# MarkJhonBao/InfantPoseEstimation_GaussianBias

Hardware: AMD Instinct MI355X
Metric: images/sec (train fwd+bwd) HRFormer-S 256x192 (higher is better)
Workload: dtype bf16; 1 GPU; HRFormer-small + fusion head, 256x192 -> 64x48, K=17, train step fwd+bwd+AdamW, DropPath 0.1, BN train; global_batch=64, per_gpu_batch=64, parallelism=dp1, launch=hipGraph replay, branches on concurrent HIP streams

## Files before the change

include/posekernels.h:

```cpp
#ifndef POSEKERNELS_H
#define POSEKERNELS_H

#include <stdint.h>

#ifdef __cplusplus
extern "C" {
#endif

#define PK_OK 0
#define PK_ERR_INVALID (-1)
#define PK_ERR_UNSUPPORTED (-2)

#define PK_DT_F32 0
#define PK_DT_BF16 1

int pk_version(void);
const char* pk_last_error_string(void);
int pk_marker(int id, void* stream);

int pk_gaussian_target(const float* keypoints, const float* visible, const float* lut, int lut_len,
                       float* target, float* weight, int B, int K, int Hh, int Wh,
                       double stride_x, double stride_y, double reach, int patch_n, int patch_c, void* stream);

int pk_dense_target(const float* keypoints, const float* visible, float* heatmaps, float* weights,
// ... 78 lines not shown



int pk_conv2d_nhwc(const void* x, const void* w_packed, void* out, float* stats_partial, const float* bias,
                   int B, int Hs, int Ws, int Cin, int Cout, int ksize, int stride, int dilated_input, int Ho, int Wo,
                   int act, int out_mode, const void* addend, void* stream);
int pk_conv2d_affine_nhwc(const void* x, const void* w_packed, void* out, const float* col_scale, const float* col_shift,
                          const void* residual, int relu, int B, int Hs, int Ws, int Cin, int Cout, int ksize, int stride, int Ho,
                          int Wo, void* stream);
int pk_conv_stats_tiles(int M);
#define PK_GROUP_MAX 12
typedef struct PkConvDesc {
    const void* x; const void* w; void* out;
    float* stats;
    const float* col_scale;
    const float* bias;
    const void* res;
    int B, Hs, Ws, Cin, Cout, ksize, stride, dilated_input, Ho, Wo;
    int act;
} PkConvDesc;
int pk_conv2d_group(const PkConvDesc* descs, int n, void* stream);
typedef struct PkBnFwdDesc {
    const void* raw; const float* stats_partial; const float* gamma; const float* beta;
    float* running_mean; float* running_var; int64_t* num_batches_tracked;
    const void* residual; void* y; float* save_mean; float* save_rstd; uint8_t* relu_mask ;
    int64_t rows; int tiles, C; float momentum, eps; int relu;
} PkBnFwdDesc;
int pk_bn_train_fwd_group(const PkBnFwdDesc* descs, int n, void* stream);
typedef struct PkBnBwdDesc {
    const void* dy; const void* y_act; const void* raw; const float* save_mean; const float* save_rstd; const float* gamma;
    float* partial; float* dgamma; float* dbeta; void* dx; void* dresidual; const uint8_t* relu_mask ;
    int64_t rows; int C; int relu;
} PkBnBwdDesc;
int pk_bn_bwd_group_blocks(int64_t rows);
int pk_bn_bwd_group(const PkBnBwdDesc* descs, int n, void* stream);
typedef struct PkFuseDesc {
    const void* inputs[4]; int in_h[4]; int in_w[4]; int n_inputs;
    void* out; const void* mask_y; int B, H, W, C, relu;
} PkFuseDesc;
int pk_fuse_sum_group(const PkFuseDesc* descs, int n, void* stream);
typedef struct PkUpBwdDesc {
    const void* dy; const void* mask_y; void* dsrc; int B, H, W, Hs, Ws, C;
} PkUpBwdDesc;
int pk_upsample_bwd_group(const PkUpBwdDesc* descs, int n, void* stream);
typedef struct PkWgradDesc {
    const void* x; const void* grad_out; float* workspace;
    int B, Hs, Ws, Ho, Wo, N, Cin, ksize, stride;
} PkWgradDesc;
int pk_wgrad_group_slices(int M, int N, int Cin, int ksize, int stride);
int pk_wgrad_group(const PkWgradDesc* descs, int n, void* stream);
int pk_sizeof_group_desc(int which);

int pk_conv_stats_rows(int B, int Hs, int Ws, int Cin, int Cout, int ksize, int stride, int Ho, int Wo);

int pk_linear_bf16(const void* x, const void* w, void* out, const float* bias, const void* residual, const float* res_scale,
                   const int32_t* a_rowmap, const int32_t* o_rowmap, void* preact_out, const void* gelu_grad_of,
                   int M, int N, int K, int rows_per_sample, int act, int out_fp32, void* stream);

int pk_rows_by_map(const void* src, void* dst, const int32_t* rowmap, int64_t n_rows, int row_bytes, int scatter, void* stream);
int pk_drop_path_f32(const float* x, const float* mask, float* out, int64_t batch, int64_t per_sample, float keep_prob, void* stream);

int pk_wgrad_slices(int M, int N, int Cin, int ksize, int stride, int Hs, int Ws, int flags);
int pk_wgrad_bf16(const void* x, const void* grad_out, float* workspace, float* dw, float* dbias, int n_bias,
                  const int32_t* a_rowmap, const int32_t* g_rowmap, const float* g_scale, int g_rows_per_sample, int M, int N,
                  int Cin, int ksize, int stride, int B, int Hs, int Ws, int Ho, int Wo, int out_layout, void* stream);

int pk_window_attn_fwd(const void* qkv, const float* rel_table, void* out, float* lse, int n_windows, int heads, int C,
                       float softmax_scale, void* stream);
int pk_window_attn_bwd_groups(int n_windows, int heads);
int pk_window_attn_bwd_ws_floats(int n_windows, int heads);
int pk_window_attn_bwd(const void* qkv, const float* rel_table, const void* fwd_out, const void* dout, const float* lse, void* dqkv,
                       float* dbias_partial, float* dtable, int n_windows, int heads, int C, float softmax_scale, void* stream);

int pk_sum_partials(const float* partial, int nb, int K, int stride, float* out, float scale, int accumulate, void* stream);
int pk_bn_finalize(const float* stats_partial, int tiles, int C, int count, const float* gamma, const float* beta,
                   float* running_mean, float* running_var, int64_t* num_batches_tracked, float momentum, float eps,
                   float* scale, float* shift, float* save_mean, float* save_rstd, void* stream);
int pk_bn_act(const void* x, const float* scale, const float* shift, const void* residual, void* y, int64_t rows, int C,
              int relu, uint8_t* relu_mask, void* stream);
int pk_bn_train_fwd(const void* raw, const float* stats_partial, int tiles, int C, int64_t rows, const float* gamma, const float* beta,
                    float* running_mean, float* running_var, int64_t* num_batches_tracked, float momentum, float eps, const void* residual,
                    void* y, float* save_mean, float* save_rstd, float* scale, float* shift, int relu, uint8_t* relu_mask, void* stream);
int pk_bn_bwd_blocks(int64_t rows);
int pk_bn_bwd(const void* dy, const void* y_act, const void* raw, const float* save_mean, const float* save_rstd,
              const float* gamma, float* partial, float* sums, float* dgamma, float* dbeta, void* dx, void* dresidual,
              int64_t rows, int C, int relu, const uint8_t* relu_mask, void* stream);
int pk_relu_bwd(const void* dy, const void* y, void* dx, int64_t numel, void* stream);
int pk_layernorm_fwd(const void* x, const float* gamma, const float* beta, void* y, float* save_mean, float* save_rstd,
                     int64_t rows, int C, int C_real, float eps, void* stream);
int pk_ln_bwd_blocks(int64_t rows);
int pk_layernorm_bwd(const void* dy, const void* x, const float* save_mean, const float* save_rstd, const float* gamma,
                     const void* dresidual, void* dx, float* partial, float* dgamma, float* dbeta, int64_t rows, int C, int C_real,
                     void* stream);
int pk_ln_mlp_supported(int C);
int pk_ln_mlp_hidden_slice(int C);
int pk_ln_mlp_slab_floats(int C);
int pk_ln_mlp_dx_blocks(int M, int C);
int pk_ln_mlp_dw_blocks(int M, int C);
int pk_ln_mlp_fwd(const void* x, const float* gamma, const float* beta, const void* w1, const float* b1, const void* w2,
                  const float* b2, const float* row_scale, void* y, int M, int C, int rows_per_sample, float eps, void* stream);
int pk_ln_mlp_wide_supported(int C, int hidden, int M);
int pk_ln_mlp_wide_fwd(const void* x, const float* gamma, const float* beta, const void* w1, const float* b1, const void* w2,
                       const float* b2, const float* row_scale, void* y, int M, int C, int c_real, int hidden, int rows_per_sample,
                       float eps, void* stream);
int pk_ln_mlp_bwd_dx(const void* dy, const void* x, const float* gamma, const float* beta, const void* w1, const float* b1,
                     const void* w1_t, const void* w2_t, const float* row_scale, void* dx, float* ln_partial, int M, int C,
// ... 51 lines not shown
```

infantposeestimation_gaussianbias_amd/nnops.py:

```python
import os

import numpy as np
import torch

from . import _lib
from ._lib import call, stream_ptr

BF16, F32, I32 = torch.bfloat16, torch.float32, torch.int32
ACT_DTYPE = BF16
WS = 7


def _e(shape, dtype, dev):
    return torch.empty(shape, dtype=dtype, device=dev)


_SINK_EPOCH = [0]


def begin_grad_epoch():
    _SINK_EPOCH[0] += 1


def sink_written(param) -> bool:
# ... 193 lines not shown
            self._dirty = True
        if self._dirty or sig != self._sig:
            call("pk_pack_weights", self.flat, self._desc, self._blk_desc, self._blk_first, self._nb, stream_ptr())
            self._sig, self._dirty = sig, False
            self.bn_eval.clear()


def weight_cache(model) -> WeightCache:
    wc = getattr(model, "_pk_weight_cache", None)
    if wc is None:
        wc = WeightCache(model)
        object.__setattr__(model, "_pk_weight_cache", wc)
    return wc


_CURRENT = []


class use_weights:
    def __init__(self, model):
        self.wc = weight_cache(model)

    def __enter__(self):
        self.wc.ensure_fresh()
        _CURRENT.append(self.wc)
        return self.wc

    def __exit__(self, *a):
        _CURRENT.pop()


def _wc():
    if not _CURRENT:
        raise _lib.PoseKernelError("nnops: no active weight cache (call the model's forward, or wrap in nnops.use_weights(model))")
    return _CURRENT[-1]


def to_features(x_nchw_f32, cpad=8):
    if x_nchw_f32.dtype == BF16 and x_nchw_f32.dim() == 4 and x_nchw_f32.shape[-1] == cpad:
        return x_nchw_f32.contiguous()
    x = x_nchw_f32.float().contiguous()
    B, Cin, H, W = x.shape
    y = _e((B, H, W, max(cpad, _up8(Cin))), BF16, x.device)
    call("pk_nchw_f32_to_nhwc_bf16", x, None, y, B, Cin, H, W, y.shape[-1], stream_ptr())
    return y


def _conv_geometry(x, ksize, stride):
    B, Hs, Ws, Cin = x.shape
    pad = ksize // 2
    return B, Hs, Ws, Cin, (Hs + 2 * pad - ksize) // stride + 1, (Ws + 2 * pad - ksize) // stride + 1


def _conv_raw(x, wf, Cout, ksize, stride, stats):
    B, Hs, Ws, Cin, Ho, Wo = _conv_geometry(x, ksize, stride)
    raw = _e((B, Ho, Wo, Cout), BF16, x.device)
    part = None
    if stats:
        tiles = _lib.lib.pk_conv_stats_rows(B, Hs, Ws, Cin, Cout, ksize, stride, Ho, Wo)
        part = _e((tiles, 2, Cout), F32, x.device)
    call("pk_conv2d_nhwc", x, wf, raw, part, None, B, Hs, Ws, Cin, Cout, ksize, stride, 0, Ho, Wo, 0, 0, None, stream_ptr())
    return raw, part


def _conv_dgrad(g, wd, Cin, ksize, stride, in_hw, addend=None):
    B, Ho, Wo, Cout = g.shape
    Hs, Ws = in_hw
    dx = _e((B, Hs, Ws, Cin), BF16, g.device)
    call("pk_conv2d_nhwc", g, wd, dx, None, None, B, Ho, Wo, Cout, Cin, ksize, 1, 1 if stride == 2 else 0, Hs, Ws, 0, 0, addend, stream_ptr())
    return dx


def _wgrad(x, g, N, Cin, ksize, stride, geom, a_map=None, g_map=None, g_scale=None, g_rps=0, M=None, oihw=True, out=None,
           dbias=None, deferred=False, win=None):
    T = ksize * ksize
    if geom is None:
        B = Hs = Ws = Ho = Wo = 0
        if win is not None:
            B, Hs, Ws = win
    else:
        B, Hs, Ws, Ho, Wo = geom
        M = B * Ho * Wo
    flags = (1 if a_map is not None else 0) | (2 if g_map is not None else 0) | (4 if g_scale is not None else 0)
    S = _lib.lib.pk_wgrad_slices(M, N, Cin, ksize, stride, Hs, Ws, flags)
    layout = 1 if (geom is not None and oihw) else 0
    n_bias = 0 if dbias is None else dbias.numel()
    if deferred and out is not None and deferral_enabled():
        ws = _workspace(out, "w", S * N * (T * Cin + 1))
        call("pk_wgrad_bf16", x, g, ws, None, None, n_bias, a_map, g_map, g_scale, g_rps, M, N, Cin, ksize, stride, B, Hs, Ws, Ho, Wo,
             layout, stream_ptr())
        total = N * T * Cin
        _defer(ws.data_ptr(), out, total, S, total, layout, N, T, Cin)
        if n_bias:
            _defer(ws.data_ptr() + 4 * S * total, dbias, N, S, n_bias)
        return out
    ws = _e((S * N * (T * Cin + 1),), F32, x.device)
    dw = out if out is not None else _e((N, Cin, ksize, ksize) if geom is not None else (N, Cin), F32, x.device)
    call("pk_wgrad_bf16", x, g, ws, dw, dbias, n_bias, a_map, g_map, g_scale, g_rps, M, N, Cin, ksize,
         stride, B, Hs, Ws, Ho, Wo, layout, stream_ptr())
    return dw


def _colsum(g, rows, N, rowmap=None, row_scale=None, rps=0, out=None):
    nb = _lib.lib.pk_ln_bwd_blocks(rows)
    part = _e((nb, N), F32, g.device)
    out = out if out is not None else _e((N,), F32, g.device)
    call("pk_colsum_bf16", g, rowmap, row_scale, rps, part, out, rows, N, stream_ptr())
    return out


class SkipGrad:
    __slots__ = ("g",)

    def __init__(self):
        self.g = None


def _bn_eval_affine(wc, bn, gamma, beta):
    key = (gamma.data_ptr(), gamma._version, beta.data_ptr(), beta._version, bn.running_mean.data_ptr(), bn.running_mean._version,
           bn.running_var.data_ptr(), bn.running_var._version)
    ent = wc.bn_eval.get(id(bn))
    if ent is None or ent[0] != key:
# ... 178 lines not shown
        dev = dy.device
        g_p, b_p = ctx.params
        (dgamma, sg), (dbeta, sb) = _sink(g_p), _sink(b_p)
        nb = _lib.lib.pk_bn_bwd_blocks(M)
        part, sums = _e((nb, 2, C), F32, dev), _e((2 * C,), F32, dev)
        draw = _e(tuple(raw.shape), BF16, dev)
        call("pk_bn_bwd", dy.contiguous(), y, raw, mean, rstd, gamma, part, sums, dgamma, dbeta, draw, None, M, C, (1 if relu else 0) | (0 if training else 2),
             None, stream_ptr())
        return draw, None, None if sg else dgamma, None if sb else dbeta, None, None, None


def deconv_bn_relu(x, deconv, bn, training):
    from . import hipops
    w = deconv.weight
    Cin, Cout, k, _ = w.shape
    if deconv.stride[0] != 2 or deconv.bias is not None or Cout % 8 or Cin % 8:
        raise _lib.PoseKernelError("deconv layer: stride-2 ConvTranspose2d without bias and channel counts that are multiples of 8")
    B, H, W, _ = x.shape
    raw_s, part = _ConvW.apply(x, _StackDeconv.apply(w))
    key = (B, H, W, str(x.device))
    if key not in _SHUFFLE_MAPS:
        b, oy, ox = torch.meshgrid(torch.arange(B), torch.arange(2 * H), torch.arange(2 * W), indexing="ij")
        m = (((b * H + oy // 2) * W + ox // 2) * 4 + (oy % 2) * 2 + (ox % 2)).reshape(-1)
        _SHUFFLE_MAPS[key] = m.to(torch.int32).to(x.device)
    raw = hipops.rows_by_map(raw_s.view(B * H * W * 4, Cout), _SHUFFLE_MAPS[key], B * 4 * H * W, False).view(B, 2 * H, 2 * W, Cout)
    t = part.shape[0]
    part4 = part.view(t, 2, 4, Cout).permute(0, 2, 1, 3).reshape(4 * t, 2, Cout).contiguous()
    return _BnActOnly.apply(raw, part4, bn.weight, bn.bias, bn, True, training)


class _HeadOut(torch.autograd.Function):
    @staticmethod
    def forward(ctx, x, weight, bias, softplus):
        ctx.params = (weight, bias)
        wc = _wc()
        wf, wd = wc.fwd[id(weight)], wc.dgrad[id(weight)]
        x = x.contiguous()
        B, H, W, Cin = x.shape
        N = weight.shape[0]
        out = _e((B, N, H, W), F32, x.device)
        call("pk_conv2d_nhwc", x, wf, out, None, bias, B, H, W, Cin, N, 1, 1, 0, H, W, 2 if softplus else 0, 2, None, stream_ptr())
        ctx.save_for_backward(x, out if softplus else x.new_empty(0), wd)
        ctx.meta = (softplus, N)
        return out

    @staticmethod
    def backward(ctx, dout):
        x, y, wd = ctx.saved_tensors
        softplus, N = ctx.meta
        B, H, W, Cin = x.shape
        Np = _up8(N)
        g = _e((B, H, W, Np), BF16, x.device)
        call("pk_nchw_f32_to_nhwc_bf16", dout.contiguous(), y if softplus else None, g, B, N, H, W, Np, stream_ptr())
        dx = _e((B, H, W, Cin), BF16, x.device)
        call("pk_conv2d_nhwc", g, wd, dx, None, None, B, H, W, Np, Cin, 1, 1, 0, H, W, 0, 0, None, stream_ptr())
        w_p, b_p = ctx.params
        dst_w, dst_b = grad_sink_of(w_p), grad_sink_of(b_p)
        if dst_w is not None and dst_b is not None and deferral_enabled():
            M = B * H * W
            S = _lib.lib.pk_wgrad_slices(M, Np, Cin, 1, 1, H, W, 0)
            ws = _workspace(dst_w, "w", S * Np * (Cin + 1))
            call("pk_wgrad_bf16", x, g, ws, None, None, N, None, None, None, 0, M, Np, Cin, 1, 1, B, H, W, H, W, 1, stream_ptr())
            _defer(ws.data_ptr(), dst_w, Np * Cin, S, N * Cin)
            _defer(ws.data_ptr() + 4 * S * Np * Cin, dst_b, Np, S, N)
            return dx, None, None, None
        db = _e((N,), F32, x.device)
        dw = _wgrad(x, g, Np, Cin, 1, 1, (B, H, W, H, W), dbias=db)[:N]
        if dst_w is not None and dst_b is not None:
            dst_w.copy_(dw)
            dst_b.copy_(db)
            return dx, None, None, None
        return dx, dw.contiguous(), db.contiguous(), None


def head_out(x, conv, softplus=False):
    return _HeadOut.apply(x, conv.weight, conv.bias, softplus)


_MAPS = {}


def window_rowmap(B, H, W, device):
    key = (B, H, W, str(device))
    if key not in _MAPS:
        nh, nw = -(-H // WS), -(-W // WS)
        ys = (torch.arange(nh)[:, None] * WS + torch.arange(WS)[None, :])
        xs = (torch.arange(nw)[:, None] * WS + torch.arange(WS)[None, :])
        yy = ys[:, None, :, None].expand(nh, nw, WS, WS)
        xx = xs[None, :, None, :].expand(nh, nw, WS, WS)
        pix = torch.where((yy < H) & (xx < W), yy * W + xx, torch.full_like(yy, -1)).reshape(-1)
        full = pix[None, :].repeat(B, 1)
        full = torch.where(full >= 0, full + torch.arange(B)[:, None] * (H * W), full)
        _MAPS[key] = (full.reshape(-1).to(torch.int32).to(device), nh * nw)
    return _MAPS[key]


def _layernorm(x2d, gamma, beta, c_real=0):
    M, C = x2d.shape
    y = _e((M, C), BF16, x2d.device)
    mean, rstd = _e((M,), F32, x2d.device), _e((M,), F32, x2d.device)
    call("pk_layernorm_fwd", x2d, gamma, beta, y, mean, rstd, M, C, c_real, 1e-5, stream_ptr())
    return y, mean, rstd


def _layernorm_bwd(dy, x2d, mean, rstd, gamma, dres, g_param=None, b_param=None, c_real=0):
    M, C = x2d.shape
    nb = _lib.lib.pk_ln_bwd_blocks(M)
    dx = _e((M, C), BF16, x2d.device)
# ... 522 lines not shown
```

infantposeestimation_gaussianbias_amd/csrc/pk_attn.hip:

```cpp
#include "pk_common.h"

typedef __attribute__((ext_vector_type(8))) short bf16x8;
typedef __attribute__((ext_vector_type(4))) float f32x4;
typedef __attribute__((ext_vector_type(4))) short s16x4;
typedef __attribute__((ext_vector_type(4))) unsigned int u32x4;

#define AT_N 49
#define AT_WS 7
#define RPITCH(DK) (32 * (DK) + 8)

__device__ __forceinline__ bf16x8 lds_frag(const uint16_t* base, int row, int pitch, int k0) {
    return *reinterpret_cast<const bf16x8*>(base + row * pitch + k0);
}
#define OOB_OFF 0x80000000u
#define MAKE_RSRC(ptr) __builtin_amdgcn_make_buffer_rsrc(const_cast<uint16_t*>(ptr), 0, 0x7ffffff0, 0x00020000)
#define GLB_FRAG(rsrc, ld, d, row, c0) \
    __builtin_bit_cast(bf16x8, __builtin_amdgcn_raw_buffer_load_b128(rsrc, ((row) < AT_N && (c0) < (d)) ? (unsigned)(((row) * (ld) + (c0)) * 2) : OOB_OFF, 0, 0))
__device__ __forceinline__ bf16x8 tok_frag(const uint16_t* tile, int pitch, int s, int col0, int lane) {
    const int g = lane >> 4, i = lane & 15;
    const uint16_t* a0 = tile + (32 * s + 4 * g + (i >> 2)) * pitch + col0 + 4 * (i & 3);
    const s16x4 lo = __builtin_amdgcn_ds_read_tr16_b64_v4i16((__attribute__((address_space(3))) s16x4*)a0);
    const s16x4 hi = __builtin_amdgcn_ds_read_tr16_b64_v4i16((__attribute__((address_space(3))) s16x4*)(a0 + 16 * pitch));
    return (bf16x8){lo[0], lo[1], lo[2], lo[3], hi[0], hi[1], hi[2], hi[3]};
}
__device__ __forceinline__ int rel_a(int t) { return 13 * (t / AT_WS) + t % AT_WS; }
__device__ __forceinline__ bf16x8 pack_frag(const f32x4 a, const f32x4 b, float m) {
    const u32x4 v = {pack_bf16x2(a[0] * m, a[1] * m), pack_bf16x2(a[2] * m, a[3] * m), pack_bf16x2(b[0] * m, b[1] * m),
                     pack_bf16x2(b[2] * m, b[3] * m)};
    return __builtin_bit_cast(bf16x8, v);
}
__device__ __forceinline__ void store4_bf16(uint16_t* dst, const f32x4 v, float m) {
    uint2 pk;
    pk.x = pack_bf16x2(v[0] * m, v[1] * m);
    pk.y = pack_bf16x2(v[2] * m, v[3] * m);
    *reinterpret_cast<uint2*>(dst) = pk;
}

#define TILE_LOAD(v, rsrc, ld, d, lane, DK)                                                                          \
    _Pragma("unroll") for (int k_ = 0; k_ < 4 * (DK); ++k_) {                                                        \
        const int idx_ = (lane) + 64 * k_, row_ = idx_ / (4 * (DK)), ch_ = idx_ % (4 * (DK));                         \
        v[k_] = __builtin_amdgcn_raw_buffer_load_b128(rsrc, (row_ < AT_N && ch_ * 8 < (d)) ? (unsigned)((row_ * (ld) + ch_ * 8) * 2) : OOB_OFF, 0, 0); \
    }
#define TILE_STORE(v, tile, lane, DK)                                                                                \
    _Pragma("unroll") for (int k_ = 0; k_ < 4 * (DK); ++k_) {                                                        \
        const int idx_ = (lane) + 64 * k_, row_ = idx_ / (4 * (DK)), ch_ = idx_ % (4 * (DK));                         \
        *reinterpret_cast<u32x4*>((tile) + row_ * RPITCH(DK) + ch_ * 8) = v[k_];                                      \
    }

template <int DK, int NCE>
__global__ void __launch_bounds__(64) k_win_attn_fwd(const uint16_t* __restrict__ qkv, const float* __restrict__ table,
                                                     uint16_t* __restrict__ out, float* __restrict__ lse, int heads, int C, int d,
                                                     float scale) {
    constexpr int RP = RPITCH(DK);
    __shared__ __attribute__((aligned(16))) uint16_t sV[64 * RP];
    __shared__ float sBias[176];
    const int lane = threadIdx.x, g4 = lane >> 4, l16 = lane & 15;
    const int w = blockIdx.x / heads, h = blockIdx.x - w * heads;
    const uint16_t* base = qkv + (size_t)w * AT_N * 3 * C + h * d;
    const auto rq = MAKE_RSRC(base), rk = MAKE_RSRC(base + C), rv = MAKE_RSRC(base + 2 * C);
    u32x4 tv[4 * DK];
    TILE_LOAD(tv, rv, 3 * C, d, lane, DK);
    bf16x8 qf[4][DK], kf[4][DK];
#pragma unroll
    for (int t = 0; t < 4; ++t)
#pragma unroll
        for (int ks = 0; ks < DK; ++ks) {
            qf[t][ks] = GLB_FRAG(rq, 3 * C, d, 16 * t + l16, 32 * ks + 8 * g4);
            kf[t][ks] = GLB_FRAG(rk, 3 * C, d, 16 * t + l16, 32 * ks + 8 * g4);
        }
    for (int i = lane; i < 169; i += 64) sBias[i] = table[i * heads + h];
    TILE_STORE(tv, sV, lane, DK);
    int aj[4][4];
#pragma unroll
    for (int cj = 0; cj < 4; ++cj)
#pragma unroll
        for (int r = 0; r < 4; ++r) {
            const int j = 16 * cj + 4 * g4 + r;
            aj[cj][r] = j < AT_N ? 84 - rel_a(j) : -1;
        }
    __syncthreads();
    bf16x8 vt[2][NCE];
#pragma unroll
    for (int s = 0; s < 2; ++s)
#pragma unroll
        for (int ce = 0; ce < NCE; ++ce) vt[s][ce] = tok_frag(sV, RP, s, 16 * ce, lane);

    const f32x4 zero = {0.f, 0.f, 0.f, 0.f};
#pragma unroll
    for (int ci = 0; ci < 4; ++ci) {
        const int i = 16 * ci + l16;
        const int ai = rel_a(i < AT_N ? i : 0);
        f32x4 st[4];
#pragma unroll
        for (int cj = 0; cj < 4; ++cj) {
            st[cj] = zero;
#pragma unroll
            for (int ks = 0; ks < DK; ++ks) st[cj] = __builtin_amdgcn_mfma_f32_16x16x32_bf16(kf[cj][ks], qf[ci][ks], st[cj], 0, 0, 0);
        }
        float mx = -INFINITY;
#pragma unroll
        for (int cj = 0; cj < 4; ++cj)
#pragma unroll
            for (int r = 0; r < 4; ++r) {
                const float bv = sBias[ai + (aj[cj][r] >= 0 ? aj[cj][r] : 0)];
                st[cj][r] = aj[cj][r] >= 0 ? st[cj][r] * scale + bv : -INFINITY;
                mx = fmaxf(mx, st[cj][r]);
            }
        mx = xor16_max(mx);
        mx = xor32_max(mx);
        float sum = 0.f;
#pragma unroll
        for (int cj = 0; cj < 4; ++cj)
#pragma unroll
            for (int r = 0; r < 4; ++r) {
                st[cj][r] = __expf(st[cj][r] - mx);
                sum += st[cj][r];
            }
        sum = xor16_sum(sum);
        sum = xor32_sum(sum);
        const float inv = 1.f / sum;
        if (g4 == 0 && i < AT_N && lse) lse[((size_t)w * heads + h) * AT_N + i] = mx + __logf(sum);
        const bf16x8 p0 = pack_frag(st[0], st[1], inv), p1 = pack_frag(st[2], st[3], inv);
#pragma unroll
        for (int ce = 0; ce < NCE; ++ce) {
            f32x4 o = __builtin_amdgcn_mfma_f32_16x16x32_bf16(vt[0][ce], p0, zero, 0, 0, 0);
            o = __builtin_amdgcn_mfma_f32_16x16x32_bf16(vt[1][ce], p1, o, 0, 0, 0);
            const int e = 16 * ce + 4 * g4;
            if (i < AT_N && e < d) store4_bf16(out + ((size_t)w * AT_N + i) * C + h * d + e, o, 1.f);
        }
    }
}

#define ATTN_DISPATCH(d, LAUNCH)            \
    do {                                    \
        if ((d) <= 16) { LAUNCH(1, 1); }    \
        else if ((d) <= 32) { LAUNCH(1, 2); } \
        else if ((d) <= 48) { LAUNCH(2, 3); } \
        else { LAUNCH(2, 4); }              \
    } while (0)

extern "C" int pk_window_attn_fwd(const void* qkv, const float* rel_table, void* out, float* lse, int n_windows, int heads, int C,
                                  float softmax_scale, void* stream) {
    PK_REQUIRE(qkv && rel_table && out && n_windows > 0 && heads > 0 && C > 0, "pk_window_attn_fwd: bad argument");
    PK_REQUIRE(C % heads == 0, "pk_window_attn_fwd: C=%d not divisible by heads=%d", C, heads);
    const int d = C / heads;
    PK_SUPPORTED(d <= 64 && (d & 7) == 0, "pk_window_attn_fwd: head_dim %d (supported: multiples of 8 up to 64)", d);
    PK_REQUIRE(((((uintptr_t)qkv) | ((uintptr_t)out)) & 15) == 0 && (C & 7) == 0, "pk_window_attn_fwd: alignment");
    const float scale = softmax_scale > 0.f ? softmax_scale : 1.f / sqrtf((float)d);
#define LAUNCH_FWD(DK_, NCE_)                                                                                                          \
    hipLaunchKernelGGL((k_win_attn_fwd<DK_, NCE_>), dim3(n_windows * heads), dim3(64), 0, (hipStream_t)stream, (const uint16_t*)qkv, \
                       rel_table, (uint16_t*)out, lse, heads, C, d, scale)
    ATTN_DISPATCH(d, LAUNCH_FWD);
#undef LAUNCH_FWD
    return pk_launch_status("pk_window_attn_fwd");
}

template <int DK, int NCE>
__global__ void __launch_bounds__(64) __attribute__((amdgpu_waves_per_eu(DK == 1 ? 2 : 1, DK == 1 ? 2 : 1))) k_win_attn_bwd(const uint16_t* __restrict__ qkv, const float* __restrict__ table,
                                                     const uint16_t* __restrict__ fwd_out, const uint16_t* __restrict__ dout,
                                                     const float* __restrict__ lse, uint16_t* __restrict__ dqkv,
                                                     float* __restrict__ dbias_part, int n_windows, int heads, int C, int d, float scale,
                                                     int wstride) {
    constexpr int RP = RPITCH(DK);
    __shared__ __attribute__((aligned(16))) uint16_t sTiles[3 * 64 * RP];
    __shared__ __attribute__((aligned(16))) float sLse[64], sDelta[64];
    __shared__ float sBias[176];
    uint16_t *sQ = sTiles, *sK = sTiles + 64 * RP, *sdO = sTiles + 2 * 64 * RP;
    const int lane0 = threadIdx.x;
    const int h = blockIdx.x % heads;
    constexpr float LOG2E = 1.44269504088896340736f;
    const float scale2 = scale * LOG2E, inv_scale = 1.f / scale;
    for (int i = lane0; i < 169; i += 64) sBias[i] = table[i * heads + h] * LOG2E;
    int a4[4][4];
#pragma unroll
    for (int c = 0; c < 4; ++c)
#pragma unroll
        for (int r = 0; r < 4; ++r) {
            const int t = 16 * c + 4 * (lane0 >> 4) + r;
            a4[c][r] = t < AT_N ? rel_a(t) : -1;
        }
    f32x4 dsum[4][4];
#pragma unroll
    for (int a = 0; a < 4; ++a)
#pragma unroll
        for (int b = 0; b < 4; ++b) dsum[a][b] = (f32x4){0.f, 0.f, 0.f, 0.f};
    const f32x4 zero = {0.f, 0.f, 0.f, 0.f};

    for (int w = blockIdx.x / heads; w < n_windows; w += wstride) {
        __syncthreads();
        const uint16_t* base = qkv + (size_t)w * AT_N * 3 * C + h * d;
        const uint16_t* dob = dout + (size_t)w * AT_N * C + h * d;
        const auto rq = MAKE_RSRC(base), rk = MAKE_RSRC(base + C), rv = MAKE_RSRC(base + 2 * C), rg = MAKE_RSRC(dob);
        const auto ro = MAKE_RSRC(fwd_out + (size_t)w * AT_N * C + h * d);
        u32x4 tq[4 * DK], tk[4 * DK], tg[4 * DK], orow[4 * DK], grow[4 * DK];
        TILE_LOAD(tq, rq, 3 * C, d, lane0, DK);
        TILE_LOAD(tk, rk, 3 * C, d, lane0, DK);
        TILE_LOAD(tg, rg, C, d, lane0, DK);
        bf16x8 vf[4][DK];
#pragma unroll
        for (int t = 0; t < 4; ++t)
#pragma unroll
            for (int ks = 0; ks < DK; ++ks) vf[t][ks] = GLB_FRAG(rv, 3 * C, d, 16 * t + (lane0 & 15), 32 * ks + 8 * (lane0 >> 4));
#pragma unroll
        for (int c = 0; c < 4 * DK; ++c) {
            const unsigned off = (lane0 < AT_N && c * 8 < d) ? (unsigned)((lane0 * C + c * 8) * 2) : OOB_OFF;
            orow[c] = __builtin_amdgcn_raw_buffer_load_b128(ro, off, 0, 0);
            grow[c] = __builtin_amdgcn_raw_buffer_load_b128(rg, off, 0, 0);
        }
        const float l = lane0 < AT_N ? lse[((size_t)w * heads + h) * AT_N + lane0] : 0.f;
        TILE_STORE(tq, sQ, lane0, DK);
        TILE_STORE(tk, sK, lane0, DK);
        TILE_STORE(tg, sdO, lane0, DK);
        {
            float de = 0.f;
#pragma unroll
            for (int c = 0; c < 4 * DK; ++c)
#pragma unroll
                for (int q = 0; q < 4; ++q) {
                    de += __uint_as_float(orow[c][q] << 16) * __uint_as_float(grow[c][q] << 16);
                    de += __uint_as_float(orow[c][q] & 0xffff0000u) * __uint_as_float(grow[c][q] & 0xffff0000u);
                }
            sLse[lane0] = -l * inv_scale;
            sDelta[lane0] = -de;
        }
        __syncthreads();
        uint16_t* dq = dqkv + (size_t)w * AT_N * 3 * C + h * d;
        int lz = 0;
        asm volatile("" : "+v"(lz));
        const int lane = lane0 + lz, g4 = lane >> 4, l16 = lane & 15;

#pragma unroll
        for (int ci = 0; ci < 4; ++ci) {
            const int i = 16 * ci + l16;
            const bool iok = ci < 3 || l16 == 0;
            const int ai = rel_a(iok ? i : 0) + 84 + lz;
            const float li = -sLse[i] * scale2, di = -sDelta[i];
            bf16x8 qfi[DK], ofi[DK];
#pragma unroll
            for (int ks = 0; ks < DK; ++ks) {
                qfi[ks] = lds_frag(sQ, i, RP, 32 * ks + g4 * 8);
                ofi[ks] = lds_frag(sdO, i, RP, 32 * ks + g4 * 8);
            }
            f32x4 acc[NCE];
#pragma unroll
            for (int ce = 0; ce < NCE; ++ce) acc[ce] = zero;
#pragma unroll
            for (int s = 0; s < 2; ++s) {
                f32x4 ds[2];
#pragma unroll
                for (int u = 0; u < 2; ++u) {
                    const int cj = 2 * s + u;
                    f32x4 sc = zero, dp = zero;
#pragma unroll
                    for (int ks = 0; ks < DK; ++ks) {
                        sc = __builtin_amdgcn_mfma_f32_16x16x32_bf16(lds_frag(sK, 16 * cj + l16, RP, 32 * ks + g4 * 8), qfi[ks], sc, 0, 0, 0);
                        dp = __builtin_amdgcn_mfma_f32_16x16x32_bf16(vf[cj][ks], ofi[ks], dp, 0, 0, 0);
                    }
#pragma unroll
                    for (int r = 0; r < 4; ++r) {
                        const bool jv = a4[cj][r] >= 0;
                        const float ev = __builtin_amdgcn_exp2f(__builtin_fmaf(sc[r], scale2, sBias[ai - (cj < 3 ? a4[cj][r] : max(a4[cj][r], 0))]) - li);
                        const float pv = (iok && jv) ? ev : 0.f;
                        ds[u][r] = pv * (dp[r] - di);
                        dsum[ci][cj][r] += ds[u][r];
                    }
                }
                const bf16x8 df = pack_frag(ds[0], ds[1], 1.f);
#pragma unroll
                for (int ce = 0; ce < NCE; ++ce)
                    acc[ce] = __builtin_amdgcn_mfma_f32_16x16x32_bf16(tok_frag(sK, RP, s, 16 * ce, lane), df, acc[ce], 0, 0, 0);
            }
#pragma unroll
            for (int ce = 0; ce < NCE; ++ce) {
                const int e = 16 * ce + 4 * g4;
                if (iok && e < d) store4_bf16(dq + (size_t)i * 3 * C + e, acc[ce], scale);
            }
        }

#pragma unroll
        for (int cj = 0; cj < 4; ++cj) {
            const int j = 16 * cj + l16;
            const bool jok = cj < 3 || l16 == 0;
            const int ajn = 84 - rel_a(jok ? j : 0) + lz;
            bf16x8 kfj[DK];
#pragma unroll
            for (int ks = 0; ks < DK; ++ks) kfj[ks] = lds_frag(sK, j, RP, 32 * ks + g4 * 8);
            f32x4 dv[NCE], dk[NCE];
#pragma unroll
            for (int ce = 0; ce < NCE; ++ce) dv[ce] = dk[ce] = zero;
#pragma unroll
            for (int s = 0; s < 2; ++s) {
                f32x4 pp[2], ds[2];
#pragma unroll
                for (int u = 0; u < 2; ++u) {
                    const int ci = 2 * s + u;
                    f32x4 sc = *reinterpret_cast<const f32x4*>(&sLse[16 * ci + 4 * g4]);
                    f32x4 dp = *reinterpret_cast<const f32x4*>(&sDelta[16 * ci + 4 * g4]);
#pragma unroll
                    for (int ks = 0; ks < DK; ++ks) {
                        sc = __builtin_amdgcn_mfma_f32_16x16x32_bf16(lds_frag(sQ, 16 * ci + l16, RP, 32 * ks + g4 * 8), kfj[ks], sc, 0, 0, 0);
                        dp = __builtin_amdgcn_mfma_f32_16x16x32_bf16(lds_frag(sdO, 16 * ci + l16, RP, 32 * ks + g4 * 8), vf[cj][ks], dp, 0, 0, 0);
                    }
#pragma unroll
                    for (int r = 0; r < 4; ++r) {
                        const bool iv = a4[ci][r] >= 0;
                        const float ev = __builtin_amdgcn_exp2f(__builtin_fmaf(sc[r], scale2, sBias[(ci < 3 ? a4[ci][r] : max(a4[ci][r], 0)) + ajn]));
                        const float pv = (jok && iv) ? ev : 0.f;
                        pp[u][r] = pv;
                        ds[u][r] = pv * dp[r];
                    }
                }
                const bf16x8 pf = pack_frag(pp[0], pp[1], 1.f), df = pack_frag(ds[0], ds[1], 1.f);
#pragma unroll
                for (int ce = 0; ce < NCE; ++ce) {
                    dv[ce] = __builtin_amdgcn_mfma_f32_16x16x32_bf16(tok_frag(sdO, RP, s, 16 * ce, lane), pf, dv[ce], 0, 0, 0);
                    dk[ce] = __builtin_amdgcn_mfma_f32_16x16x32_bf16(tok_frag(sQ, RP, s, 16 * ce, lane), df, dk[ce], 0, 0, 0);
                }
            }
#pragma unroll
            for (int ce = 0; ce < NCE; ++ce) {
                const int e = 16 * ce + 4 * g4;
                if (jok && e < d) {
                    store4_bf16(dq + (size_t)j * 3 * C + C + e, dk[ce], scale);
                    store4_bf16(dq + (size_t)j * 3 * C + 2 * C + e, dv[ce], 1.f);
                }
            }
        }
    }
    __syncthreads();
    static_assert((320 + 6 * 7 * AT_N + 12 * AT_N + AT_N) * 4 <= 3 * 64 * RP * 2, "bias-gradient tile + slack must fit the Q/K/dO tiles");
    float* sD = reinterpret_cast<float*>(sTiles) + 320;
#pragma unroll
    for (int ci = 0; ci < 4; ++ci)
#pragma unroll
        for (int cj = 0; cj < 4; ++cj)
#pragma unroll
            for (int r = 0; r < 4; ++r) {
                const int i = 16 * ci + (lane0 & 15), j = 16 * cj + 4 * (lane0 >> 4) + r;
                if (i < AT_N && j < AT_N) sD[i * AT_N + j] = dsum[ci][cj][r];
            }
    __syncthreads();
    for (int e = lane0; e < 169; e += 64) {
        const int dy = e / 13 - 6, dx = e % 13 - 6;
        const int x0 = max(0, -dx), x1 = min(AT_WS, AT_WS - dx);
        unsigned keep[AT_WS];
#pragma unroll
        for (int xj = 0; xj < AT_WS; ++xj) keep[xj] = (xj >= x0 && xj < x1) ? 0xffffffffu : 0u;
        const int base = (dy * AT_WS + dx) * AT_N;
        float acc = 0.f;
        for (int yj = max(0, -dy); yj < min(AT_WS, AT_WS - dy); ++yj) {
#pragma unroll
            for (int xj = 0; xj < AT_WS; ++xj) {
                const float v = sD[base + yj * (AT_WS * AT_N + AT_WS) + xj * (AT_N + 1)];
                acc += __uint_as_float(__float_as_uint(v) & keep[xj]);
            }
        }
        dbias_part[(size_t)blockIdx.x * 169 + e] = acc;
    }
}

__global__ void __launch_bounds__(256) k_relbias_reduce(const float* __restrict__ part, int n_groups, int heads, float* __restrict__ dtable) {
    __shared__ float sh[256];
    const int e = blockIdx.x, h = blockIdx.y, t = threadIdx.x;
    const int per_head = n_groups / heads;
    float s = 0.f;
    for (int k = t; k < per_head; k += 256) s += part[(size_t)(k * heads + h) * 169 + e];
    sh[t] = s;
    __syncthreads();
#pragma unroll
// ... 39 lines not shown
```

Measured before the change: 4250 images/sec.

## Add persistent panel kernel for thin-K 1x1 convolutions with register-resident weights

Adds a specialized HIP kernel for 1x1 stride-1 convolutions with small input channels (K<=64) and 128/256 outputs. It keeps the whole weight slice in registers, runs a persistent grid of 64-row panels with next-panel prefetch, and optionally fuses BN partial statistics or a residual addend. It is routed from forward conv, dgrad, and the head dgrad when M is large enough. The aim is to avoid the generic conv kernel's overhead on these bandwidth-bound shapes, at the cost of higher register pressure and a separate stats-row layout.

New measurement: 4268 images/sec, median of 2. About the same (+0.4%).

```diff
diff --git a/include/posekernels.h b/include/posekernels.h
--- a/include/posekernels.h
+++ b/include/posekernels.h
@@ -154,6 +154,11 @@
 int pk_sizeof_group_desc(int which);
 
 int pk_conv_stats_rows(int B, int Hs, int Ws, int Cin, int Cout, int ksize, int stride, int Ho, int Wo);
+
+int pk_conv1x1_panel(const void* x, const void* w, void* out, float* stats, const void* addend, int M, int K, int N, void* stream);
+int pk_conv1x1_panel_supported(int M, int K, int N);
+int pk_conv1x1_panel_stats_rows(int M, int N);
+int pk_conv1x1_panel_tile_rows(void);
 
 int pk_linear_bf16(const void* x, const void* w, void* out, const float* bias, const void* residual, const float* res_scale,
                    const int32_t* a_rowmap, const int32_t* o_rowmap, void* preact_out, const void* gelu_grad_of,
diff --git a/infantposeestimation_gaussianbias_amd/csrc/pk_conv1x1p.hip b/infantposeestimation_gaussianbias_amd/csrc/pk_conv1x1p.hip
--- /dev/null
+++ b/infantposeestimation_gaussianbias_amd/csrc/pk_conv1x1p.hip
@@ -0,0 +1,174 @@
+#include "pk_common.h"
+
+#define P1_ROWS 64
+#define P1_WG_PER_CU 2
+
+__device__ __forceinline__ float p1_bf16_lo(uint32_t u) { return __uint_as_float(u << 16); }
+__device__ __forceinline__ float p1_bf16_hi(uint32_t u) { return __uint_as_float(u & 0xffff0000u); }
+
+template <int N, int KS, int MODE>
+__global__ void __launch_bounds__(256, 2) k_conv1x1p(const uint16_t* __restrict__ x, const uint16_t* __restrict__ w, uint16_t* __restrict__ out,
+                                                     float* __restrict__ stats, const uint16_t* __restrict__ addend, int M, int K) {
+    constexpr int WC = N / 4, NT = WC / 16, NQ = NT / 2, NB = P1_ROWS / 16;
+    const int tid = threadIdx.x, lane = tid & 63;
+    const int wave = __builtin_amdgcn_readfirstlane(tid >> 6);
+    const int p = lane & 15, g = lane >> 4;
+    const int npanels = (M + P1_ROWS - 1) / P1_ROWS;
+    int first, step, n_mine;
+    {
+        const int G = gridDim.x, L = blockIdx.x, q = npanels >> 3, r = npanels & 7, xl = L & 7, j = L >> 3;
+        const int start = xl < r ? xl * (q + 1) : r * (q + 1) + (xl - r) * q, cnt = q + (xl < r ? 1 : 0);
+        step = (G - xl + 7) >> 3;
+        first = start + j;
+        n_mine = j < cnt ? (cnt - j + step - 1) / step : 0;
+    }
+    const auto rx = __builtin_amdgcn_make_buffer_rsrc(const_cast<uint16_t*>(x), 0, 0x7ffffff0, 0x00020000);
+    const auto rw = __builtin_amdgcn_make_buffer_rsrc(const_cast<uint16_t*>(w), 0, 0x7ffffff0, 0x00020000);
+    const auto ro = __builtin_amdgcn_make_buffer_rsrc(out, 0, 0x7ffffff0, 0x00020000);
+    const auto ra = __builtin_amdgcn_make_buffer_rsrc(const_cast<uint16_t*>(MODE == 2 ? addend : x), 0, 0x7ffffff0, 0x00020000);
+
+    auto load_panel = [&](int panel, bf16x8 (&a)[NB][KS]) {
+#pragma unroll
+        for (int b = 0; b < NB; ++b) {
+            const int m = panel * P1_ROWS + b * 16 + p;
+#pragma unroll
+            for (int ks = 0; ks < KS; ++ks) {
+                const int k = ks * 32 + g * 8;
+                unsigned off = (m < M && k < K) ? (unsigned)(m * K + k) * 2u : OOB_OFF;
+                asm volatile("" : "+v"(off));
+                a[b][ks] = __builtin_bit_cast(bf16x8, __builtin_amdgcn_raw_buffer_load_b128(rx, off, 0, 0));
+            }
+        }
+    };
+    bf16x8 cur[NB][KS], nxt[NB][KS];
+    if (n_mine > 0) load_panel(first, cur);
+    bf16x8 wreg[KS][NT];
+#pragma unroll
+    for (int ks = 0; ks < KS; ++ks)
+#pragma unroll
+        for (int a = 0; a < NT; ++a) {
+            const int n = wave * WC + (a >> 1) * 32 + 8 * (p >> 2) + 4 * (a & 1) + (p & 3), k = ks * 32 + g * 8;
+            const unsigned off = k < K ? (unsigned)(n * K + k) * 2u : OOB_OFF;
+            wreg[ks][a] = __builtin_bit_cast(bf16x8, __builtin_amdgcn_raw_buffer_load_b128(rw, off, 0, 0));
+        }
+#pragma unroll
+    for (int ks = 0; ks < KS; ++ks) {
+#pragma unroll
+        for (int a = 0; a < NT; ++a) asm volatile("s_waitcnt vmcnt(0)" : "+v"(wreg[ks][a])::"memory");
+#pragma unroll
+        for (int b = 0; b < NB; ++b) asm volatile("s_waitcnt vmcnt(0)" : "+v"(cur[b][ks])::"memory");
+    }
+    float ssum[NT][4], ssq[NT][4];
+#pragma unroll
+    for (int a = 0; a < NT; ++a)
+#pragma unroll
+        for (int r = 0; r < 4; ++r) ssum[a][r] = ssq[a][r] = 0.f;
+
+    for (int it = 0; it < n_mine; ++it) {
+        const int panel = first + it * step;
+        if (it + 1 < n_mine) load_panel(panel + step, nxt);
+        f32x4 acc[NT][NB];
+#pragma unroll
+        for (int a = 0; a < NT; ++a)
+#pragma unroll
+            for (int b = 0; b < NB; ++b) acc[a][b] = (f32x4){0.f, 0.f, 0.f, 0.f};
+#pragma unroll
+        for (int ks = 0; ks < KS; ++ks)
+#pragma unroll
+            for (int b = 0; b < NB; ++b)
+#pragma unroll
+                for (int a = 0; a < NT; ++a) acc[a][b] = __builtin_amdgcn_mfma_f32_16x16x32_bf16(wreg[ks][a], cur[b][ks], acc[a][b], 0, 0, 0);
+#pragma unroll
+        for (int b = 0; b < NB; ++b) {
+            const int m = panel * P1_ROWS + b * 16 + p;
+#pragma unroll
+            for (int q = 0; q < NQ; ++q) {
+                const unsigned off = m < M ? (unsigned)(m * N + wave * WC + q * 32 + 8 * g) * 2u : OOB_OFF;
+                const f32x4 lo = acc[2 * q][b], hi = acc[2 * q + 1][b];
+                if (MODE == 1) {
+#pragma unroll
+                    for (int r = 0; r < 4; ++r) {
+                        ssum[2 * q][r] += lo[r];
+                        ssq[2 * q][r] += lo[r] * lo[r];
+                        ssum[2 * q + 1][r] += hi[r];
+                        ssq[2 * q + 1][r] += hi[r] * hi[r];
+                    }
+                }
+                float v[8] = {lo[0] + 0.f, lo[1] + 0.f, lo[2] + 0.f, lo[3] + 0.f, hi[0] + 0.f, hi[1] + 0.f, hi[2] + 0.f, hi[3] + 0.f};
+                if (MODE == 2) {
+                    const u32x4 rv = __builtin_amdgcn_raw_buffer_load_b128(ra, off, 0, 0);
+#pragma unroll
+                    for (int j = 0; j < 4; ++j) {
+                        v[2 * j] += p1_bf16_lo(rv[j]);
+                        v[2 * j + 1] += p1_bf16_hi(rv[j]);
+                    }
+                }
+                const u32x4 o = {pack_bf16x2(v[0], v[1]), pack_bf16x2(v[2], v[3]), pack_bf16x2(v[4], v[5]), pack_bf16x2(v[6], v[7])};
+                __builtin_amdgcn_raw_buffer_store_b128(o, ro, off, 0, 0);
+            }
+        }
+        if (it + 1 < n_mine) {
+#pragma unroll
+            for (int b = 0; b < NB; ++b)
+#pragma unroll
+                for (int ks = 0; ks < KS; ++ks) cur[b][ks] = nxt[b][ks];
+        }
+    }
+    if (MODE == 1) {
+        float* dst = stats + (size_t)blockIdx.x * 2 * N;
+#pragma unroll
+        for (int a = 0; a < NT; ++a)
+#pragma unroll
+            for (int r = 0; r < 4; ++r) {
+                const float sm = lanes_sum<16>(ssum[a][r]), sq = lanes_sum<16>(ssq[a][r]);
+                if (p == 0) {
+                    const int ch = wave * WC + (a >> 1) * 32 + 8 * g + 4 * (a & 1) + r;
+                    dst[ch] = sm;
+                    dst[N + ch] = sq;
+                }
+            }
+    }
+}
+
+static inline int p1_cu_count() {
+    static int cus = 0;
+    int dev = 0, n = 0;
+    if (!cus) cus = (hipGetDevice(&dev) != hipSuccess || hipDeviceGetAttribute(&n, hipDeviceAttributeMultiprocessorCount, dev) != hipSuccess || n <= 0) ? 256 : n;
+    return cus;
+}
+static inline int p1_grid(int M) {
+    const long npanels = ((long)M + P1_ROWS - 1) / P1_ROWS, cap = (long)P1_WG_PER_CU * p1_cu_count();
+    return (int)(npanels < cap ? npanels : cap);
+}
+static inline bool p1_shape_ok(int K, int N) { return K >= 8 && K <= 64 && (K % 8) == 0 && (N == 128 || N == 256); }
+
+extern "C" int pk_conv1x1_panel_tile_rows(void) { return P1_ROWS; }
+extern "C" int pk_conv1x1_panel_supported(int M, int K, int N) {
+    return p1_shape_ok(K, N) && M > 0 && (long)M >= 2L * P1_ROWS * P1_WG_PER_CU * p1_cu_count() && (long)M * N < 0x3fffffffL;
+}
+extern "C" int pk_conv1x1_panel_stats_rows(int M, int N) { return (M > 0 && (N == 128 || N == 256)) ? p1_grid(M) : 0; }
+
+#define P1_LAUNCH(N_, KS_, MODE_)                                                                                                         \
+    hipLaunchKernelGGL((k_conv1x1p<N_, KS_, MODE_>), dim3((unsigned)p1_grid(M)), dim3(256), 0, (hipStream_t)stream, (const uint16_t*)x,   \
+                       (const uint16_t*)w, (uint16_t*)out, stats, (const uint16_t*)addend, M, K)
+#define P1_MODES(N_, KS_)                     \
+    switch (mode) {                           \
+    case 0: P1_LAUNCH(N_, KS_, 0); break;     \
+    case 1: P1_LAUNCH(N_, KS_, 1); break;     \
+    default: P1_LAUNCH(N_, KS_, 2); break;    \
+    }
+extern "C" int pk_conv1x1_panel(const void* x, const void* w, void* out, float* stats, const void* addend, int M, int K, int N, void* stream) {
+    PK_REQUIRE(x && w && out, "pk_conv1x1_panel: null pointer");
+    PK_REQUIRE(M > 0, "pk_conv1x1_panel: bad size M=%d", M);
+    PK_SUPPORTED(p1_shape_ok(K, N), "pk_conv1x1_panel: built for K %% 8 == 0, K <= 64 and N = 128 / 256, got K=%d N=%d", K, N);
+    PK_REQUIRE((((uintptr_t)x | (uintptr_t)w | (uintptr_t)out | (uintptr_t)addend) & 15) == 0, "pk_conv1x1_panel: pointers must be 16-byte aligned");
+    PK_REQUIRE((int64_t)M * N < 0x3fffffffLL, "pk_conv1x1_panel: tensor too large for 32-bit byte offsets");
+    PK_REQUIRE(!(stats && addend), "pk_conv1x1_panel: statistics go with the plain output only (as in pk_conv2d_nhwc)");
+    const int mode = stats ? 1 : (addend ? 2 : 0);
+    if (N == 256) {
+        if (K > 32) { P1_MODES(256, 2) } else { P1_MODES(256, 1) }
+    } else {
+        if (K > 32) { P1_MODES(128, 2) } else { P1_MODES(128, 1) }
+    }
+    return pk_launch_status("pk_conv1x1_panel");
+}
diff --git a/infantposeestimation_gaussianbias_amd/nnops.py b/infantposeestimation_gaussianbias_amd/nnops.py
--- a/infantposeestimation_gaussianbias_amd/nnops.py
+++ b/infantposeestimation_gaussianbias_amd/nnops.py
@@ -269,10 +269,19 @@
     return B, Hs, Ws, Cin, (Hs + 2 * pad - ksize) // stride + 1, (Ws + 2 * pad - ksize) // stride + 1
 
 
+def _panel_route(M, K, N):
+    return os.environ.get("PK_CONV1X1P", "1") != "0" and _lib.lib.pk_conv1x1_panel_supported(M, K, N) == 1
+
+
 def _conv_raw(x, wf, Cout, ksize, stride, stats):
     B, Hs, Ws, Cin, Ho, Wo = _conv_geometry(x, ksize, stride)
     raw = _e((B, Ho, Wo, Cout), BF16, x.device)
     part = None
+    if ksize == 1 and stride == 1 and _panel_route(B * Ho * Wo, Cin, Cout):
+        if stats:
+            part = _e((_lib.lib.pk_conv1x1_panel_stats_rows(B * Ho * Wo, Cout), 2, Cout), F32, x.device)
+        call("pk_conv1x1_panel", x, wf, raw, part, None, B * Ho * Wo, Cin, Cout, stream_ptr())
+        return raw, part
     if stats:
         tiles = _lib.lib.pk_conv_stats_rows(B, Hs, Ws, Cin, Cout, ksize, stride, Ho, Wo)
         part = _e((tiles, 2, Cout), F32, x.device)
@@ -284,7 +293,20 @@
     B, Ho, Wo, Cout = g.shape
     Hs, Ws = in_hw
     dx = _e((B, Hs, Ws, Cin), BF16, g.device)
+    if ksize == 1 and stride == 1 and _panel_route(B * Hs * Ws, Cout, Cin):
+        call("pk_conv1x1_panel", g, wd, dx, None, addend, B * Hs * Ws, Cout, Cin, stream_ptr())
+        return dx
     call("pk_conv2d_nhwc", g, wd, dx, None, None, B, Ho, Wo, Cout, Cin, ksize, 1, 1 if stride == 2 else 0, Hs, Ws, 0, 0, addend, stream_ptr())
+    return dx
+
+
+def _head_dgrad(g, wd, Cin):
+    B, H, W, Np = g.shape
+    dx = _e((B, H, W, Cin), BF16, g.device)
+    if _panel_route(B * H * W, Np, Cin):
+        call("pk_conv1x1_panel", g, wd, dx, None, None, B * H * W, Np, Cin, stream_ptr())
+    else:
+        call("pk_conv2d_nhwc", g, wd, dx, None, None, B, H, W, Np, Cin, 1, 1, 0, H, W, 0, 0, None, stream_ptr())
     return dx
 
 
@@ -569,8 +591,7 @@
         Np = _up8(N)
         g = _e((B, H, W, Np), BF16, x.device)
         call("pk_nchw_f32_to_nhwc_bf16", dout.contiguous(), y if softplus else None, g, B, N, H, W, Np, stream_ptr())
-        dx = _e((B, H, W, Cin), BF16, x.device)
-        call("pk_conv2d_nhwc", g, wd, dx, None, None, B, H, W, Np, Cin, 1, 1, 0, H, W, 0, 0, None, stream_ptr())
+        dx = _head_dgrad(g, wd, Cin)
         w_p, b_p = ctx.params
         dst_w, dst_b = grad_sink_of(w_p), grad_sink_of(b_p)
         if dst_w is not None and dst_b is not None and deferral_enabled():
```

## Swizzle window-attention LDS tiles and keep row fragments in registers

Applied to the files above, without the earlier changes.

Replaces the padded-pitch LDS tile layout in the window-attention forward and backward kernels with an XOR-swizzled unpadded layout, for both row-fragment and transposed reads, to cut bank conflicts and LDS footprint. The backward kernel now loads Q/K/dO straight into MFMA row fragments and writes them to LDS from those. For DK==2 it keeps them in registers rather than re-reading LDS. It also sets an occupancy hint for the DK==2 forward kernel. Keeping the fragments in registers raises VGPR pressure and may cause spills or lower occupancy.

Result: no change. 4246 images/sec before, 4231 images/sec after, median of 2 (-0.4%).

```diff
diff --git a/infantposeestimation_gaussianbias_amd/csrc/pk_attn.hip b/infantposeestimation_gaussianbias_amd/csrc/pk_attn.hip
--- a/infantposeestimation_gaussianbias_amd/csrc/pk_attn.hip
+++ b/infantposeestimation_gaussianbias_amd/csrc/pk_attn.hip
@@ -7,20 +7,20 @@
 
 #define AT_N 49
 #define AT_WS 7
-#define RPITCH(DK) (32 * (DK) + 8)
-
-__device__ __forceinline__ bf16x8 lds_frag(const uint16_t* base, int row, int pitch, int k0) {
-    return *reinterpret_cast<const bf16x8*>(base + row * pitch + k0);
-}
+#define TPITCH(DK) (32 * (DK))
+template <int DK> constexpr __device__ __forceinline__ int tile_swz(int row) { return ((row * DK) >> 1) & (4 * DK - 1); }
+template <int DK> constexpr __device__ __forceinline__ int tile_off(int row, int chunk) { return row * TPITCH(DK) + 8 * (chunk ^ tile_swz<DK>(row)); }
 #define OOB_OFF 0x80000000u
 #define MAKE_RSRC(ptr) __builtin_amdgcn_make_buffer_rsrc(const_cast<uint16_t*>(ptr), 0, 0x7ffffff0, 0x00020000)
 #define GLB_FRAG(rsrc, ld, d, row, c0) \
     __builtin_bit_cast(bf16x8, __builtin_amdgcn_raw_buffer_load_b128(rsrc, ((row) < AT_N && (c0) < (d)) ? (unsigned)(((row) * (ld) + (c0)) * 2) : OOB_OFF, 0, 0))
-__device__ __forceinline__ bf16x8 tok_frag(const uint16_t* tile, int pitch, int s, int col0, int lane) {
+template <int DK>
+__device__ __forceinline__ bf16x8 tok_frag(const uint16_t* tile, int s, int col0, int lane) {
+    static_assert(tile_swz<DK>(16) == 0 && (8 * DK & (4 * DK - 1)) == 0, "the swizzle must repeat 16 rows down");
     const int g = lane >> 4, i = lane & 15;
-    const uint16_t* a0 = tile + (32 * s + 4 * g + (i >> 2)) * pitch + col0 + 4 * (i & 3);
+    const uint16_t* a0 = tile + tile_off<DK>(32 * s + 4 * g + (i >> 2), (col0 >> 3) + ((i >> 1) & 1)) + 4 * (i & 1);
     const s16x4 lo = __builtin_amdgcn_ds_read_tr16_b64_v4i16((__attribute__((address_space(3))) s16x4*)a0);
-    const s16x4 hi = __builtin_amdgcn_ds_read_tr16_b64_v4i16((__attribute__((address_space(3))) s16x4*)(a0 + 16 * pitch));
+    const s16x4 hi = __builtin_amdgcn_ds_read_tr16_b64_v4i16((__attribute__((address_space(3))) s16x4*)(a0 + 16 * TPITCH(DK)));
     return (bf16x8){lo[0], lo[1], lo[2], lo[3], hi[0], hi[1], hi[2], hi[3]};
 }
 __device__ __forceinline__ int rel_a(int t) { return 13 * (t / AT_WS) + t % AT_WS; }
@@ -44,15 +44,14 @@
 #define TILE_STORE(v, tile, lane, DK)                                                                                \
     _Pragma("unroll") for (int k_ = 0; k_ < 4 * (DK); ++k_) {                                                        \
         const int idx_ = (lane) + 64 * k_, row_ = idx_ / (4 * (DK)), ch_ = idx_ % (4 * (DK));                         \
-        *reinterpret_cast<u32x4*>((tile) + row_ * RPITCH(DK) + ch_ * 8) = v[k_];                                      \
+        *reinterpret_cast<u32x4*>((tile) + tile_off<DK>(row_, ch_)) = v[k_];                                          \
     }
 
 template <int DK, int NCE>
-__global__ void __launch_bounds__(64) k_win_attn_fwd(const uint16_t* __restrict__ qkv, const float* __restrict__ table,
+__global__ void __launch_bounds__(64) __attribute__((amdgpu_waves_per_eu(DK == 2 ? 4 : 1))) k_win_attn_fwd(const uint16_t* __restrict__ qkv, const float* __restrict__ table,
                                                      uint16_t* __restrict__ out, float* __restrict__ lse, int heads, int C, int d,
                                                      float scale) {
-    constexpr int RP = RPITCH(DK);
-    __shared__ __attribute__((aligned(16))) uint16_t sV[64 * RP];
+    __shared__ __attribute__((aligned(16))) uint16_t sV[64 * TPITCH(DK)];
     __shared__ float sBias[176];
     const int lane = threadIdx.x, g4 = lane >> 4, l16 = lane & 15;
     const int w = blockIdx.x / heads, h = blockIdx.x - w * heads;
@@ -83,7 +82,7 @@
 #pragma unroll
     for (int s = 0; s < 2; ++s)
 #pragma unroll
-        for (int ce = 0; ce < NCE; ++ce) vt[s][ce] = tok_frag(sV, RP, s, 16 * ce, lane);
+        for (int ce = 0; ce < NCE; ++ce) vt[s][ce] = tok_frag<DK>(sV, s, 16 * ce, lane);
 
     const f32x4 zero = {0.f, 0.f, 0.f, 0.f};
 #pragma unroll
@@ -161,7 +160,8 @@
                                                      const float* __restrict__ lse, uint16_t* __restrict__ dqkv,
                                                      float* __restrict__ dbias_part, int n_windows, int heads, int C, int d, float scale,
                                                      int wstride) {
-    constexpr int RP = RPITCH(DK);
+    constexpr int RP = TPITCH(DK);
+    constexpr bool ROWREG = DK == 2;
     __shared__ __attribute__((aligned(16))) uint16_t sTiles[3 * 64 * RP];
     __shared__ __attribute__((aligned(16))) float sLse[64], sDelta[64];
     __shared__ float sBias[176];
@@ -192,15 +192,18 @@
         const uint16_t* dob = dout + (size_t)w * AT_N * C + h * d;
         const auto rq = MAKE_RSRC(base), rk = MAKE_RSRC(base + C), rv = MAKE_RSRC(base + 2 * C), rg = MAKE_RSRC(dob);
         const auto ro = MAKE_RSRC(fwd_out + (size_t)w * AT_N * C + h * d);
-        u32x4 tq[4 * DK], tk[4 * DK], tg[4 * DK], orow[4 * DK], grow[4 * DK];
-        TILE_LOAD(tq, rq, 3 * C, d, lane0, DK);
-        TILE_LOAD(tk, rk, 3 * C, d, lane0, DK);
-        TILE_LOAD(tg, rg, C, d, lane0, DK);
-        bf16x8 vf[4][DK];
+        u32x4 orow[4 * DK], grow[4 * DK];
+        bf16x8 qf[4][DK], kf[4][DK], gf[4][DK], vf[4][DK];
 #pragma unroll
         for (int t = 0; t < 4; ++t)
 #pragma unroll
-            for (int ks = 0; ks < DK; ++ks) vf[t][ks] = GLB_FRAG(rv, 3 * C, d, 16 * t + (lane0 & 15), 32 * ks + 8 * (lane0 >> 4));
+            for (int ks = 0; ks < DK; ++ks) {
+                const int row = 16 * t + (lane0 & 15), c0 = 32 * ks + 8 * (lane0 >> 4);
+                qf[t][ks] = GLB_FRAG(rq, 3 * C, d, row, c0);
+                kf[t][ks] = GLB_FRAG(rk, 3 * C, d, row, c0);
+                gf[t][ks] = GLB_FRAG(rg, C, d, row, c0);
+                vf[t][ks] = GLB_FRAG(rv, 3 * C, d, row, c0);
+            }
 #pragma unroll
         for (int c = 0; c < 4 * DK; ++c) {
             const unsigned off = (lane0 < AT_N && c * 8 < d) ? (unsigned)((lane0 * C + c * 8) * 2) : OOB_OFF;
@@ -208,9 +211,15 @@
             grow[c] = __builtin_amdgcn_raw_buffer_load_b128(rg, off, 0, 0);
         }
         const float l = lane0 < AT_N ? lse[((size_t)w * heads + h) * AT_N + lane0] : 0.f;
-        TILE_STORE(tq, sQ, lane0, DK);
-        TILE_STORE(tk, sK, lane0, DK);
-        TILE_STORE(tg, sdO, lane0, DK);
+#pragma unroll
+        for (int t = 0; t < 4; ++t)
+#pragma unroll
+            for (int ks = 0; ks < DK; ++ks) {
+                const int off = tile_off<DK>(16 * t + (lane0 & 15), 4 * ks + (lane0 >> 4));
+                *reinterpret_cast<bf16x8*>(sQ + off) = qf[t][ks];
+                *reinterpret_cast<bf16x8*>(sK + off) = kf[t][ks];
+                *reinterpret_cast<bf16x8*>(sdO + off) = gf[t][ks];
+            }
         {
             float de = 0.f;
 #pragma unroll
@@ -225,6 +234,10 @@
         }
         __syncthreads();
         uint16_t* dq = dqkv + (size_t)w * AT_N * 3 * C + h * d;
+#define ROW_FRAG(reg, tile, t, ks) (ROWREG ? reg[t][ks] : *reinterpret_cast<const bf16x8*>(tile + tile_off<DK>(16 * (t) + l16, 4 * (ks) + g4)))
+#define ROW_Q(t, ks) ROW_FRAG(qf, sQ, t, ks)
+#define ROW_K(t, ks) ROW_FRAG(kf, sK, t, ks)
+#define ROW_G(t, ks) ROW_FRAG(gf, sdO, t, ks)
         int lz = 0;
         asm volatile("" : "+v"(lz));
         const int lane = lane0 + lz, g4 = lane >> 4, l16 = lane & 15;
@@ -237,10 +250,7 @@
             const float li = -sLse[i] * scale2, di = -sDelta[i];
             bf16x8 qfi[DK], ofi[DK];
 #pragma unroll
-            for (int ks = 0; ks < DK; ++ks) {
-                qfi[ks] = lds_frag(sQ, i, RP, 32 * ks + g4 * 8);
-                ofi[ks] = lds_frag(sdO, i, RP, 32 * ks + g4 * 8);
-            }
+            for (int ks = 0; ks < DK; ++ks) qfi[ks] = ROW_Q(ci, ks), ofi[ks] = ROW_G(ci, ks);
             f32x4 acc[NCE];
 #pragma unroll
             for (int ce = 0; ce < NCE; ++ce) acc[ce] = zero;
@@ -253,7 +263,7 @@
                     f32x4 sc = zero, dp = zero;
 #pragma unroll
                     for (int ks = 0; ks < DK; ++ks) {
-                        sc = __builtin_amdgcn_mfma_f32_16x16x32_bf16(lds_frag(sK, 16 * cj + l16, RP, 32 * ks + g4 * 8), qfi[ks], sc, 0, 0, 0);
+                        sc = __builtin_amdgcn_mfma_f32_16x16x32_bf16(ROW_K(cj, ks), qfi[ks], sc, 0, 0, 0);
                         dp = __builtin_amdgcn_mfma_f32_16x16x32_bf16(vf[cj][ks], ofi[ks], dp, 0, 0, 0);
                     }
 #pragma unroll
@@ -268,7 +278,7 @@
                 const bf16x8 df = pack_frag(ds[0], ds[1], 1.f);
 #pragma unroll
                 for (int ce = 0; ce < NCE; ++ce)
-                    acc[ce] = __builtin_amdgcn_mfma_f32_16x16x32_bf16(tok_frag(sK, RP, s, 16 * ce, lane), df, acc[ce], 0, 0, 0);
+                    acc[ce] = __builtin_amdgcn_mfma_f32_16x16x32_bf16(tok_frag<DK>(sK, s, 16 * ce, lane), df, acc[ce], 0, 0, 0);
             }
 #pragma unroll
             for (int ce = 0; ce < NCE; ++ce) {
@@ -284,7 +294,7 @@
             const int ajn = 84 - rel_a(jok ? j : 0) + lz;
             bf16x8 kfj[DK];
 #pragma unroll
-            for (int ks = 0; ks < DK; ++ks) kfj[ks] = lds_frag(sK, j, RP, 32 * ks + g4 * 8);
+            for (int ks = 0; ks < DK; ++ks) kfj[ks] = ROW_K(cj, ks);
             f32x4 dv[NCE], dk[NCE];
 #pragma unroll
             for (int ce = 0; ce < NCE; ++ce) dv[ce] = dk[ce] = zero;
@@ -298,8 +308,8 @@
                     f32x4 dp = *reinterpret_cast<const f32x4*>(&sDelta[16 * ci + 4 * g4]);
 #pragma unroll
                     for (int ks = 0; ks < DK; ++ks) {
-                        sc = __builtin_amdgcn_mfma_f32_16x16x32_bf16(lds_frag(sQ, 16 * ci + l16, RP, 32 * ks + g4 * 8), kfj[ks], sc, 0, 0, 0);
-                        dp = __builtin_amdgcn_mfma_f32_16x16x32_bf16(lds_frag(sdO, 16 * ci + l16, RP, 32 * ks + g4 * 8), vf[cj][ks], dp, 0, 0, 0);
+                        sc = __builtin_amdgcn_mfma_f32_16x16x32_bf16(ROW_Q(ci, ks), kfj[ks], sc, 0, 0, 0);
+                        dp = __builtin_amdgcn_mfma_f32_16x16x32_bf16(ROW_G(ci, ks), vf[cj][ks], dp, 0, 0, 0);
                     }
 #pragma unroll
                     for (int r = 0; r < 4; ++r) {
@@ -313,8 +323,8 @@
                 const bf16x8 pf = pack_frag(pp[0], pp[1], 1.f), df = pack_frag(ds[0], ds[1], 1.f);
 #pragma unroll
                 for (int ce = 0; ce < NCE; ++ce) {
-                    dv[ce] = __builtin_amdgcn_mfma_f32_16x16x32_bf16(tok_frag(sdO, RP, s, 16 * ce, lane), pf, dv[ce], 0, 0, 0);
-                    dk[ce] = __builtin_amdgcn_mfma_f32_16x16x32_bf16(tok_frag(sQ, RP, s, 16 * ce, lane), df, dk[ce], 0, 0, 0);
+                    dv[ce] = __builtin_amdgcn_mfma_f32_16x16x32_bf16(tok_frag<DK>(sdO, s, 16 * ce, lane), pf, dv[ce], 0, 0, 0);
+                    dk[ce] = __builtin_amdgcn_mfma_f32_16x16x32_bf16(tok_frag<DK>(sQ, s, 16 * ce, lane), df, dk[ce], 0, 0, 0);
                 }
             }
 #pragma unroll
```
